# yutiansut/marl-optimal-execution

Measured on AMD Instinct MI355X. Metric: env-steps/sec (whole node), rmsc03 100-agent market ×4096 envs, 1/2/4/8 GPUs, higher is better.
Workload: dtype int64; 1 GPU; rmsc03 x4096 envs per GPU, full episode per step (config build from seeds + the config's session), seeds 123456789+global_env; envs_per_gpu=4096, global_envs=4096, parallelism=envs sharded, dp1, parity_hash=False, env_errors=0, agents_per_env=64, device=AMD Radeon Graphics, cus=256

## Files before the change

### include/mxa.h

```cpp
#ifndef MXA_H
#define MXA_H
#include <stdint.h>
#ifdef __cplusplus
extern "C" {
#endif

typedef struct mxa_handle mxa_handle;

enum { MXA_RMSC03 = 0, MXA_SPARSE_ZI_100 = 1, MXA_SPARSE_ZI_1000 = 2, MXA_MARKETREPLAY = 3, MXA_RMSC03_RL = 4,
       MXA_VALUE_NOISE = 5 ,
       MXA_RMSC01 = 6 ,
       MXA_RMSC02 = 7 ,
       MXA_OBI_RMSC02 = 8 ,
       MXA_RANDOM_FUND_VALUE = 9 ,
       MXA_RANDOM_FUND_DIVERSE = 10 ,
       MXA_HIST_FUND_VALUE = 11 ,
       MXA_HIST_FUND_DIVERSE = 12 ,
       MXA_MARKETREPLAY_RUNNER = 13 ,
       MXA_MARKETREPLAY_TWAP = 14 ,
       MXA_RMSC03_SBMM = 15, MXA_RMSC03_SBMM_POLL = 16,
       MXA_RMSC03_MM = 17 };
enum {
  MXA_OK = 0, MXA_EINVAL = -1, MXA_EHIP = -2, MXA_ENOMEM = -3, MXA_ERANGE = -4
};
// ... 124 lines not shown
  const float* params; int32_t n_layers; int32_t dims[9];
  const double* grid0; int32_t n0; const double* grid1; int32_t n1;
  double nh, q0;
  const double* table;
  int32_t test, enough;
  const double* u; const int64_t* rnd;
  const double* eps;
} mxa_policy;
int mxa_step_policy(mxa_handle* h, int32_t k, int32_t first_zero, const mxa_policy* p, double* d_obs,
                    int32_t* d_flags, int64_t* d_a, double* d_act, double* d_state);
int mxa_set_parity_hash(mxa_handle* h, int32_t enabled);
#define MXA_RL_STATE_WORDS 8
int mxa_write_rl_state(mxa_handle* h, double* device_out);
const char* mxa_build_id(void);

typedef struct {
  int64_t t;
  int32_t price;
  int32_t qty;
} mxa_book_rec;
#define MXA_BL_FUNDAMENTAL (-2147483647 - 1)
int mxa_set_book_log(mxa_handle* h, int32_t cap);
#define MXA_BL_EV_RX (-2147483647 - 1 + 256)
#define MXA_BL_EV_NT (MXA_BL_EV_RX + 256)
#define MXA_BL_EV_PLACE (MXA_BL_EV_RX + 512)
#define MXA_BL_EV_END (MXA_BL_EV_RX + 768)
int mxa_set_exchange_log(mxa_handle* h, int32_t on);
int mxa_read_book_log(mxa_handle* h, int32_t env, mxa_book_rec* out, int64_t cap, int64_t* n);

#include "mxa_snap.h"
#include "mxa_depth.h"
#include "mxa_bars.h"
#include "mxa_variates.h"
#include "mxa_policy_features.h"

int mxa_rng_probe(int32_t device, uint32_t seed, int32_t mode, double a, double b, int32_t n, double* out);
int mxa_math_probe(int32_t device, int32_t mode, const double* x, const double* y, double* out, int64_t n);
int mxa_policy_probe(void* stream, int32_t n, const float* x, const float* params, int32_t n_layers,
                     const int32_t* dims, int32_t test, int32_t enough, const double* u, const int64_t* rnd,
                     const double* eps, float* q, int64_t* a);

#ifdef __cplusplus
}
#endif
#endif
```

### marl-optimal-execution_amd/build_lib.py

```python
import hashlib
import os
import subprocess
import sys
from concurrent.futures import ThreadPoolExecutor

HERE = os.path.dirname(os.path.abspath(__file__))
ROOT = os.path.dirname(HERE)
SRC = os.path.join(HERE, "csrc", "mxa_api.hip")
INST = os.path.join(HERE, "csrc", "mxa_inst.hip")
OUT = os.path.join(HERE, "lib", "libmxa.so")
OBJ = os.path.join(HERE, "build")
N_CONFIGS = 18
DEPS = ["mxa_api.hip", "mxa_inst.hip", "mxa_entry.h", "mxa_kernels.hip", "mxa_layout.h", "mxa_config.h", "glibc_math.h",
        "glibc_math_tables.h", "qnet_wave_device.h", "ddqn_device.h", "mxa_snapshot.h", "mxa_depth_kernels.h",
        "mxa_bars_kernels.h"]
HIPCC = os.environ.get("HIPCC", "/opt/rocm/bin/hipcc")
FLAGS = ["--offload-arch=gfx950", "-O3", "-std=c++20", "-ffp-contract=off", "-fno-fast-math", "-fPIC", "-shared",
         "-Wno-unused-result", "-Wno-unused-value", "-mllvm", "-structurizecfg-skip-uniform-regions"]

CFG_FLAGS = {1: ["-mllvm", "-amdgpu-sched-strategy=max-ilp"], 2: ["-fno-slp-vectorize"],
             3: ["-mllvm", "-amdgpu-sched-strategy=max-ilp"]}


def sources():
    return [os.path.join(HERE, "csrc", d) for d in DEPS] + [os.path.join(ROOT, "include", h) for h in ("mxa.h", "mxa_snap.h", "mxa_depth.h", "mxa_bars.h", "mxa_variates.h", "mxa_policy_features.h", "mxa_state_spec.h")]


def build_id(extra=()):
    h = hashlib.sha256()
    for s in sources():
        with open(s, "rb") as f:
            h.update(f.read())
    h.update(" ".join(FLAGS + list(extra)).encode())
    h.update(repr(sorted(CFG_FLAGS.items())).encode())
    return h.hexdigest()[:16]


def up_to_date():
    if not os.path.exists(OUT):
        return False
    t = os.path.getmtime(OUT)
    return all(os.path.getmtime(s) <= t for s in sources() + [os.path.abspath(__file__)])


def build(force=False, verbose=True, jobs=None):
    if not force and up_to_date():
        return OUT
    os.makedirs(os.path.dirname(OUT), exist_ok=True)
    os.makedirs(OBJ, exist_ok=True)
    inc = ["-I" + os.path.join(HERE, "csrc"), "-I" + os.path.join(ROOT, "include")]
    cflags = [f for f in FLAGS if f != "-shared"] + ["-c"]
    jit = ['-DMXA_JIT_FLAGS="%s"' % " ".join(FLAGS),
           '-DMXA_JIT_CFG_FLAGS="%s"' % ";".join("%d:%s" % (c, " ".join(f)) for c, f in sorted(CFG_FLAGS.items()))]
    units = [([HIPCC] + cflags + ['-DMXA_BUILD_ID="%s"' % build_id()] + jit + inc + [SRC, "-o", os.path.join(OBJ, "mxa_api.o")])]
    for c in range(N_CONFIGS):
        units.append([HIPCC] + cflags + CFG_FLAGS.get(c, []) + ["-DMXA_INST_CFG=%d" % c] + inc +
                     [INST, "-o", os.path.join(OBJ, "mxa_inst_%d.o" % c)])
    if verbose:
# ... 41 lines not shown
```

### marl-optimal-execution_amd/csrc/mxa_api.hip

```cpp
#include <hip/hip_runtime.h>

#include <dlfcn.h>
#include <spawn.h>
#include <sys/stat.h>
#include <sys/wait.h>
#include <unistd.h>

#include <algorithm>
#include <cstddef>
#include <cstdio>
#include <cstdlib>
#include <cstring>
#include <map>
#include <memory>
#include <mutex>
#include <string>
#include <vector>

extern char** environ;

#include "../../include/mxa.h"
#define MXA_API_TU
#include "mxa_kernels.hip"
#include "mxa_entry.h"
// ... 1239 lines not shown
  if (n <= 0 || !out || mode < 0 || mode > 5) return MXA_EINVAL;
  if (hipSetDevice(device) != hipSuccess) return MXA_EHIP;
  DevBuf<double> d_out;
  DevBuf<uint32_t> d_s;
  if (d_out.alloc(n) != hipSuccess || d_s.alloc(MXA_RNG_WORDS) != hipSuccess) return MXA_ENOMEM;
  hipLaunchKernelGGL(mxa_rng_probe_kernel, dim3(1), dim3(64), 0, 0, seed, mode, a, b, n, d_out.p, d_s.p);
  if (hipGetLastError() != hipSuccess) return MXA_EHIP;
  return hipMemcpy(out, d_out, sizeof(double) * n, hipMemcpyDeviceToHost) == hipSuccess ? MXA_OK : MXA_EHIP;
}

int mxa_variate_probe(int32_t device, uint32_t seed, const uint8_t* script, int32_t n, int32_t lookahead, double* out,
                      uint64_t* state) {
  if (n <= 0 || !script || !out || !state || lookahead < 2 || lookahead > 256) return MXA_EINVAL;
  for (int32_t i = 0; i < n; i++)
    if (script[i] > 3) return MXA_EINVAL;
  if (hipSetDevice(device) != hipSuccess) return MXA_EHIP;
  DevBuf<uint8_t> d_script;
  DevBuf<double> d_out;
  DevBuf<uint64_t> d_state, d_tab;
  DevBuf<uint32_t> d_s;
  if (d_script.alloc(n) != hipSuccess || d_out.alloc(2 * (size_t)n) != hipSuccess || d_state.alloc(6 * (size_t)n) != hipSuccess ||
      d_tab.alloc(MXA_VT_BYTES / 8) != hipSuccess || d_s.alloc(2 * MXA_RNG_WORDS) != hipSuccess)
    return MXA_ENOMEM;
  if (hipMemcpy(d_script, script, (size_t)n, hipMemcpyHostToDevice) != hipSuccess ||
      hipMemset(d_tab, 0, MXA_VT_BYTES) != hipSuccess)
    return MXA_EHIP;
  hipLaunchKernelGGL(mxa_variate_probe_kernel, dim3(1), dim3(64), 0, 0, seed, d_script.p, n, lookahead, d_out.p, d_state.p,
                     d_s.p, d_tab.p);
  if (hipGetLastError() != hipSuccess) return MXA_EHIP;
  if (hipMemcpy(out, d_out, sizeof(double) * 2 * (size_t)n, hipMemcpyDeviceToHost) != hipSuccess) return MXA_EHIP;
  return hipMemcpy(state, d_state, sizeof(uint64_t) * 6 * (size_t)n, hipMemcpyDeviceToHost) == hipSuccess ? MXA_OK : MXA_EHIP;
}

int mxa_math_probe(int32_t device, int32_t mode, const double* x, const double* y, double* out, int64_t n) {
  if (n <= 0 || !x || !out) return MXA_EINVAL;
  if (hipSetDevice(device) != hipSuccess) return MXA_EHIP;
  DevBuf<double> dx, dy, dout;
  size_t bytes = sizeof(double) * n;
  if (dx.alloc(n) != hipSuccess || dy.alloc(n) != hipSuccess || dout.alloc(n) != hipSuccess) return MXA_ENOMEM;
  if (hipMemcpy(dx, x, bytes, hipMemcpyHostToDevice) != hipSuccess ||
      hipMemcpy(dy, y ? y : x, bytes, hipMemcpyHostToDevice) != hipSuccess)
    return MXA_EHIP;
  hipLaunchKernelGGL(mxa_math_probe_kernel, dim3((unsigned)((n + 255) / 256)), dim3(256), 0, 0, mode, dx.p, dy.p, dout.p,
                     n);
  if (hipGetLastError() != hipSuccess) return MXA_EHIP;
  return hipMemcpy(out, dout, bytes, hipMemcpyDeviceToHost) == hipSuccess ? MXA_OK : MXA_EHIP;
}

int mxa_policy_probe(void* stream, int32_t n, const float* x, const float* params, int32_t n_layers, const int32_t* dims,
                     int32_t test, int32_t enough, const double* u, const int64_t* rnd, const double* eps, float* q,
                     int64_t* a) {
  if (n <= 0 || !x || !params || !qwave::dims_ok(n_layers, dims) || (!q && !a)) return MXA_EINVAL;
  if (a && !test && (!u || !rnd || !eps)) return MXA_EINVAL;
  MxaPolicyProbe p{};
  p.params = params;
  p.n_layers = n_layers;
  for (int i = 0; i <= n_layers; i++) p.dims[i] = dims[i];
  p.test = test;
  p.enough = enough;
  p.u = u;
  p.rnd = rnd;
  p.eps = eps;
  hipLaunchKernelGGL(mxa_policy_probe_kernel, dim3((unsigned)n), dim3(64), 0, (hipStream_t)stream, p, n, x, q, a);
  return hipGetLastError() == hipSuccess ? MXA_OK : MXA_EHIP;
}

// ... 219 lines not shown
```

### marl-optimal-execution_amd/csrc/mxa_config.h

```cpp
#pragma once
#include <stddef.h>
#include "mxa_layout.h"
#include "../../include/mxa.h"

namespace mxa_cfg {

constexpr int64_t NS = 1000000000LL;
constexpr int64_t MIN = 60 * NS;
constexpr int64_t HOUR = 60 * MIN;

struct Shape {
  int sq, so;
  bool pl;
  int waves;
  int pw;
  int hot;
  int sql = 0;
};
constexpr int sq_lds(int cfg);
constexpr int lat_lds(int cfg);
constexpr Shape shape(int cfg);
constexpr bool is_custom(int cfg);
#ifndef MXA_RMSC03_WAVES
#define MXA_RMSC03_WAVES 4
// ... 79 lines not shown
       : (cfg == MXA_CFG_RANDOM_FUND_VALUE || cfg == MXA_CFG_HIST_FUND_VALUE) ? Shape{96, 5, false, MXA_RFV_WAVES, 6, 0, MXA_RFV_SQL}
       : (cfg == MXA_CFG_RANDOM_FUND_DIVERSE || cfg == MXA_CFG_HIST_FUND_DIVERSE)
           ? Shape{96, MXA_SO_RFD, false, MXA_RFD_WAVES, 8, 0, MXA_RFD_SQL}
                                       : Shape{4, 1, true, 2, 8, MXA_RP_HOT};
}
constexpr int sq_lds(int cfg) { return shape(cfg).sql ? shape(cfg).sql : shape(cfg).sq; }
constexpr bool rp_hdr_lds(int cfg) {
  return cfg == MXA_CFG_MARKETREPLAY || cfg == MXA_CFG_MARKETREPLAY_RUNNER || cfg == MXA_CFG_MARKETREPLAY_TWAP;
}
#ifndef MXA_BOOK_LDS_RFV
#define MXA_BOOK_LDS_RFV 0x34
#endif
constexpr int book_lds(int cfg) {
  return cfg == MXA_CFG_RMSC02 ? MXA_BOOK_LDS_RMSC02
         : (cfg >= MXA_CFG_RANDOM_FUND_VALUE && cfg <= MXA_CFG_HIST_FUND_DIVERSE) ? MXA_BOOK_LDS_RFV
                                                                                 : 0;
}
#ifndef MXA_TEMPER_FILL_MASK
#define MXA_TEMPER_FILL_MASK ((1 << MXA_CFG_RMSC03) | (1 << MXA_CFG_SPARSE_ZI_100) | (1 << MXA_CFG_VALUE_NOISE))
#endif
#ifndef MXA_ONE_ADVANCE_MASK
#define MXA_ONE_ADVANCE_MASK MXA_TEMPER_FILL_MASK
#endif
constexpr bool temper_fill(int cfg) { return (((MXA_TEMPER_FILL_MASK) >> cfg) & 1) != 0; }
constexpr bool one_advance(int cfg) { return (((MXA_ONE_ADVANCE_MASK) >> cfg) & 1) != 0; }
#ifndef MXA_VARIATE_O_MASK
#define MXA_VARIATE_O_MASK (1 << MXA_CFG_RMSC03)
#endif
#ifndef MXA_VARIATE_AGENT_MASK
#define MXA_VARIATE_AGENT_MASK (1 << MXA_CFG_RMSC03)
#endif
constexpr bool variate_o(int cfg) { return (((MXA_VARIATE_O_MASK) >> cfg) & 1) != 0 && !is_custom(cfg); }
constexpr bool variate_agent(int cfg) { return (((MXA_VARIATE_AGENT_MASK) >> cfg) & 1) != 0 && !is_custom(cfg); }
#define MXA_VT_O_BYTES ((2 * 64 + 2) * 8)
#define MXA_VT_BYTES 2048
constexpr size_t lds_bytes(int cfg) {
  return (size_t)sq_lds(cfg) * 64 * (12 + (shape(cfg).pl ? 4 * shape(cfg).pw : 0)) + 512
         + (size_t)shape(cfg).hot * 512
         + 1024
         + (variate_o(cfg) ? MXA_VT_O_BYTES : 0)
         + (size_t)lat_lds(cfg) * 8
         + (rp_hdr_lds(cfg) ? 256 : 0)
         + (size_t)__builtin_popcount(book_lds(cfg)) * shape(cfg).so * 256
         + 256
#ifdef MXA_PROF
         + 1024
#endif
      ;
}

constexpr void base_params(MxaParams& P) {
  P.o_rbar = 1e5;
  P.o_kappa = 1.67e-12;
  P.o_fundvol = 1e-4;
  P.o_lambda = 2.77778e-13;
  P.o_msmean = 1e3;
  P.o_msvar = 5e4;
  P.starting_cash = 10000000;
  P.ex_pipeline = 0;
  P.ex_comp = 0;
  P.stream_history = 10;
  P.mkt_open = 9 * HOUR + 30 * MIN;
}

constexpr void params_rmsc03(MxaParams& P) {
  base_params(P);
// ... 736 lines not shown
```

### marl-optimal-execution_amd/csrc/mxa_kernels.hip

```cpp
#pragma once
#include <hip/hip_runtime.h>
#if defined(MXA_ONLY_RMSC03) && !(defined(MXA_ONLY_CFG) && (MXA_ONLY_CFG == 3 || MXA_ONLY_CFG == 4))
#define MXA_NO_GYM
#endif

#ifndef MXA_HINT_MASK
#define MXA_HINT_MASK ((1 << 0) | (1 << 4))
#endif
#if defined(MXA_INST_CFG)
#define MXA_HINT_ON (((MXA_HINT_MASK) >> (MXA_INST_CFG)) & 1)
#elif defined(MXA_ONLY_RMSC03) && defined(MXA_ONLY_CFG)
#define MXA_HINT_ON (((MXA_HINT_MASK) >> (MXA_ONLY_CFG)) & 1)
#elif defined(MXA_ONLY_RMSC03)
#define MXA_HINT_ON ((MXA_HINT_MASK) & 1)
#else
#define MXA_HINT_ON 0
#endif
#define MXA_EXPECT_(x, v) __builtin_expect(!!(x), v)
#define MXA_PROB_(x, v, p) __builtin_expect_with_probability(!!(x), v, p)
#if MXA_HINT_ON
#define MXA_LIKELY(x) MXA_EXPECT_(x, 1)
#define MXA_UNLIKELY(x) MXA_EXPECT_(x, 0)
#define MXA_RARE(x) MXA_EXPECT_(x, 0)
#define MXA_RARE_P(x, p) MXA_PROB_(x, 1, p)
// ... 188 lines not shown
      a1[q][k] = ok ? A[i + 1] : 0u;
      if (ph == 0) a3[q][k] = ok ? A[i + 397] : 0u;
    }
    a623[q] = on ? A[623] : 0u;
  }
#pragma unroll
  for (int q = 0; q < 2; q++) {
    if (q == 1 && !two) break;
    u32* B = key[q] + (bb[q] & 1) * MXA_MT_N;
    u32 y[11];
#pragma unroll
    for (int k = 0; k < 4; k++) y[k] = a3[q][k] ^ mt_mix(a0[q][k], a1[q][k]);
#pragma unroll
    for (int k = 4; k < 11; k++) y[k] = y[k - 4] ^ mt_mix(a0[q][k], a1[q][k]);
    const u32 b396 = rdl(y[6], 41), b0 = rdl(y[0], 0);
#pragma unroll
    for (int k = 0; k < 11; k++) {
      const int ph = k < 4 ? 0 : k < 8 ? 1 : 2, kk = k - 4 * ph;
      if (kk * 64 + lane < (ph < 2 ? 227 : 169)) B[227 * ph + lane + 64 * kk] = y[k];
    }
    if (lane == 0) B[623] = b396 ^ mt_mix(a623[q], b0);
  }
  wfence();
}
DEV void mt_gen_build(u32* key, int b) { mt_gen_pair(key, b, key, b, false); }

DEV void mt_seed(u32* key, u32 s) {
  const int lane = laneid();
  for (int i = 0; i < MXA_MT_N; i++) {
    if ((i & 63) == lane) key[i] = s;
    s = 1812433253u * (s ^ (s >> 30)) + (u32)i + 1u;
  }
  wfence();
}

DEV u32 mt_temper(u32 y) {
  y ^= (y >> 11);
  y ^= (y << 7) & 0x9d2c5680u;
  y ^= (y << 15) & 0xefc60000u;
  y ^= (y >> 18);
  return y;
}
template <bool B, int W, bool TF>
DEV void rs_fill(RSt<B, W, TF>& r) {
  const int lane = laneid();
  const int q = r.p + lane, b = q / MXA_MT_N;
  const bool ok = b <= r.m && b >= r.m - 1;
  u32 v = 0;
  if (ok) v = r.key[(b & 1) * MXA_MT_N + (q - b * MXA_MT_N)];
  if constexpr (TF) v = mt_temper(v);
  r.lw[lane] = v;
  const u64 okb = __ballot(ok);
  r.lwn = ~okb == 0 ? 64 : __ffsll((unsigned long long)~okb) - 1;
  r.lw0 = r.p;
  if (r.lwn == 0) r.hasg |= 2;
  __threadfence_block();
}
template <bool B, int W, bool TF>
DEV u32 rs_u32(RSt<B, W, TF>& r) {
  if constexpr (W == RS_WIN || W == RS_PTR) {
    if (W == RS_WIN || r.lw) {
      u32 off = (u32)(r.p - r.lw0);
      if (MXA_RARE(off >= (u32)r.lwn)) {
        if constexpr (B) {
          const int blk = r.p / MXA_MT_N;
          while (r.m < blk) {
// ... 2182 lines not shown
    __threadfence_block();
    rs(AF_NUSED, (u32)base);
    return base;
  }

  DEV bool ta_wakeup() {
    PROF_SCOPE(75);
    u32 f = flags();
    if (f & FL_FIRST_WAKE) rs(AF_FLAGS, f & ~FL_FIRST_WAKE);
    if (!(f & FL_HAS_OPEN)) {
      send_ex(msg_make(MK_WHEN_OPEN_REQ, cur_agent));
      send_ex(msg_make(MK_WHEN_CLOSE_REQ, cur_agent));
    }
    f = flags();
    return (f & FL_HAS_OPEN) && (f & FL_HAS_CLOSE) && !(f & FL_MKT_CLOSED);
  }
  DEV i64 wake_frequency(int type) {
    if (type == AG_POVMM) return mm_wake();
    if (type == AG_MOMENTUM) return PC.mom_wake;
    if (type == AG_MKTMAKER) return PC.mk_wake;
    if (type == AG_OBI) return PC.obi_wake;
    if (type == AG_SBMM) return PC.sb_wake;
    if constexpr (RP) {
      if (type == AG_REPLAY) return U(rx->tm[0]) - PC.mkt_open;
      if constexpr (TW) {
        if (type == AG_TWAP) return PC.rl_h0 - PC.mkt_open;
      }
    }
    if constexpr (GYM) {
      if (type == AG_DUMMYRL) return PC.rl_h0 - PC.mkt_open;
    }
    ARS A = agent_rs();
    i64 v = rs_randint(A, 0, 100);
    agent_rs_put(A);
    return v;
  }
  DEV void query_last_trade(const Msg& m) {
    u32 f = flags() | FL_HAS_LAST;
    f = m_dfloat(m) ? (f | FL_LAST_FLOAT) : (f & ~FL_LAST_FLOAT);
    if (f & FL_MKT_CLOSED) f |= FL_DAILY_CLOSE;
    rs(AF_FLAGS, f);
    rs64(AF_LAST_TRADE, (i64)(i32)m.w[5]);
  }
  DEV void ta_receive(const Msg& m, int type) {
    PROF_SCOPE(74);
    u32 f0 = flags();
    bool had = (f0 & FL_HAS_OPEN) && (f0 & FL_HAS_CLOSE);
    switch (m_kind(m)) {
    case MK_WHEN_OPEN:
      rs64(AF_MKT_OPEN, m_i64(m, 1));
      fl_set(FL_HAS_OPEN, true);
      break;
    case MK_WHEN_CLOSE:
      rs64(AF_MKT_CLOSE, m_i64(m, 1));
      fl_set(FL_HAS_CLOSE, true);
      break;
    case MK_EXECUTED: {
      i64 q = m_buy(m) ? (i64)(i32)m.w[2] : -(i64)(i32)m.w[2];
      rs64(AF_SHARES, rg64(AF_SHARES) + q);
      rs64(AF_CASH, rg64(AF_CASH) - q * (i64)(i32)m.w[4]);
      if constexpr (RP) {
        if (type == AG_REPLAY) {
          RPCHK((i32)m.w[5] >= 0 && (i32)m.w[5] < U(rx->L.D), "ta_receive EXECUTED dense", (i32)m.w[5]);
          RpOrder* o = mro() + (i32)m.w[5];
          const RpOrder ov = *o;
          if (U(ov.present)) {
// ... 2742 lines not shown
    this->rs(AF_FLAGS, FL_FIRST_WAKE | FL_AW_SPREAD | FL_AW_TV);
    this->rs(AF_RS_POS, MXA_MT_N);
    this->rs(AF_RS_M, 0);
    const i64 cash = type == AG_VALUE ? E::PC.v_starting_cash : E::PC.starting_cash;
    this->rs64(AF_START_CASH, cash);
    this->rs64(AF_CASH, cash);
    this->rs64(AF_ATIME, E::PC.start);
    this->rs64(AF_COMP, E::PC.default_comp_delay);
  }
  DEV i64 get_wake_time(RS& G, i64 open, i64 close) { return wake_time_of(rs_double(G), open, close); }
  DEV void wake_times_lanes() {
    const MxaParams& P = E::PC;
    wfence();
    for (int a0 = P.first_noise; a0 < P.first_noise + P.n_noise; a0 += 64) {
      const int a = a0 + this->lane;
      if (a < P.first_noise + P.n_noise) {
        u32* rw = (u32*)this->agent_ptr(a);
        const double u = as_d(((u64)rw[AF_WAKEUP_TIME + 1] << 32) | rw[AF_WAKEUP_TIME]);
        const u64 wt = (u64)wake_time_of(u, P.noise_open, P.noise_close);
        rw[AF_WAKEUP_TIME] = (u32)wt;
        rw[AF_WAKEUP_TIME + 1] = (u32)(wt >> 32);
      }
    }
    wfence();
  }
  DEV i64 wake_time_of(double u, i64 open, i64 close) {
    double alpha = 12.0, beta = 0.5;
    double n = (3 / alpha) * u - gm_pow(beta - 0, 3.0);
    double c = n < 0 ? -gm_pow(-n, 1.0 / 3.0) : gm_pow(n, 1.0 / 3.0);
    double mult = c + beta;
    return open + (i64)(mult * (double)(close - open));
  }
  static constexpr bool SEED_TILE = E::LDS_Q >= 64 * 17 * 4;
  DEV void seed_streams(int first) {
    const MxaParams& P = E::PC;
    wfence();
    const int lane = this->lane;
    for (int b = first; b < P.n_streams; b += 64) {
      int s = b + lane;
      if constexpr (SEED_TILE) {
        LDSP u32* tile = (LDSP u32*)this->qk;
        u32 x = s < P.n_streams ? this->rng_key(s)[0] : 0u;
        for (int i0 = 1; i0 < MXA_MT_N; i0 += 16) {
#pragma unroll
          for (int j = 0; j < 16; j++) {
            x = 1812433253u * (x ^ (x >> 30)) + (u32)(i0 + j);
            tile[lane * 17 + j] = x;
          }
          __builtin_amdgcn_wave_barrier();
#pragma unroll
          for (int t = 0; t < 16; t++) {
            const int st = 4 * t + (lane >> 4), w = lane & 15;
            if (b + st < P.n_streams && i0 + w < MXA_MT_N) this->rng_key(b + st)[i0 + w] = tile[st * 17 + w];
          }
          __builtin_amdgcn_wave_barrier();
        }
      } else if (s < P.n_streams) {
        u32* key = this->rng_key(s);
        u32 x = key[0];
        for (int i = 1; i < MXA_MT_N; i++) {
          x = 1812433253u * (x ^ (x >> 30)) + (u32)i;
          key[i] = x;
        }
      }
    }
    wfence();
    if constexpr (SEED_TILE) {
      for (int j = 0; j < E::SQ; j++) this->qset(j, KEY_EMPTY, 0xFFFFFFFFu, true);
      if constexpr (E::QHIER) this->q_rescan();
    }
  }

  DEV void maint_agents() {
    const int n = E::PC.n_agents, lane = this->lane;
    wfence();
    for (int a0 = 0; a0 < n; a0 += 64) {
      const int a = a0 + lane;
      const bool act = a < n;
      u32* rw = (u32*)this->agent_ptr(act ? a : a0);
      const i32 p = act ? (i32)rw[AF_RS_POS] : 0;
      i32 m = act ? (i32)rw[AF_RS_M] : 0;
      const i32 need = (p + MXA_AGENT_LA) / MXA_MT_N;
      for (;;) {
        u64 t = bal(act && m < need);
        if (!t) break;
        const int l1 = ctz64(t);
        t &= t - 1;
        const int l2 = t ? ctz64(t) : l1;
        const int m1 = rdl((u32)m, l1), m2 = rdl((u32)m, l2);
        mt_gen_pair(this->rng_key(4 + a0 + l1), m1 + 1, this->rng_key(4 + a0 + l2), m2 + 1, l2 != l1);
        m += (lane == l1 || lane == l2) ? 1 : 0;
      }
      if (act) rw[AF_RS_M] = (u32)m;
    }
    wfence();
  }

  u64 zi_fb[(E::PC.n_zi + E::PC.n_hbl + 63) / 64 + 1];
  DEV bool zi_fallback(int a) {
    const int i = a - E::PC.first_zi;
    return (zi_fb[i >> 6] >> (i & 63)) & 1;
  }
  DEV void zi_theta_lanes() {
    const MxaParams& P = E::PC;
    constexpr int NQ = 2 * E::PC.zi_qmax;
    static_assert(NQ <= 20, "theta fits the agent record");
    const int lo = P.first_zi, hi = P.first_zi + P.n_zi + P.n_hbl;
    const double sd = __builtin_sqrt(P.zi_sigma_pv);
    const int lane = this->lane;
    for (int a0 = lo; a0 < hi; a0 += 64) {
      for (int j = 0; j < 64 && a0 + j < hi; j += 2)
        mt_gen_pair(this->rng_key(4 + a0 + j), 1, this->rng_key(4 + a0 + j + 1), 1, a0 + j + 1 < hi);
      const int a = a0 + lane;
      const bool act = a < hi;
      const u32* key = this->rng_key(4 + (act ? a : a0));
      i32 p = MXA_MT_N;
      bool cached = false, fb = false;
// ... 389 lines not shown
      double* lat = this->lat();
      i64 total = (i64)n * n, prev = -1;
      bool col = P.config == MXA_CFG_SPARSE_ZI_100;
      i64 nneed = col ? 2 * (i64)n - 1 : (i64)n;
      for (i64 k = 0; k < nneed; k++) {
        i64 d = k < n ? k : (k - n + 1) * (i64)n;
        rs_skip_words(G, 2 * (d - prev - 1));
        double v = rs_uniform(G, P.lat_lo, P.lat_hi);
        if (this->lane == 0) {
          if (d < n) lat[d] = v;
          if (col && d % n == 0) lat[n + d / n] = v;
        }
        prev = d;
      }
      rs_skip_words(G, 2 * (total - prev - 1));
      if (P.config == MXA_CFG_SPARSE_ZI_1000) {
        if (this->lane == 0) lat[0] = 20000.0;
      }
      wfence();
    }
    this->grs_put(0, G);
    seed_streams(1);
    h.rs_pos[1] = h.rs_pos[2] = h.rs_pos[3] = MXA_MT_N;
    h.rs_m[1] = h.rs_m[2] = h.rs_m[3] = 0;
    if constexpr (!E::EXT) {
      RS O = this->grs(1);
      double msv = rs_normal(O, P.o_msmean, __builtin_sqrt(P.o_msvar));
      h.o_msv = rs_randint(O, 0, 2) == 0 ? msv : -msv;
      this->grs_put(1, O);
    }
    rec_init(0, AG_EXCHANGE);
    this->rs64(AF_COMP, P.default_comp_delay);
    this->rec_store();
    for (int a = P.first_mom; a < P.first_mom + P.n_mom; a++) {
      this->rec_load(a);
      ARS A = this->agent_rs();
      this->rs(AF_SIZE, (u32)rs_randint(A, P.mom_min, P.mom_max));
      this->agent_rs_put(A);
      this->rec_store();
    }
    for (int a = P.first_mk; a < P.first_mk + P.n_mk; a++) {
      this->rec_load(a);
      ARS A = this->agent_rs();
      this->rs(AF_SIZE, (u32)(i64)__builtin_rint((double)rs_randint(A, P.mk_min, P.mk_max) / 2));
      this->agent_rs_put(A);
      this->rec_store();
    }
    constexpr bool ZI_LANES = E::PC.n_zi + E::PC.n_hbl > 0;
    if constexpr (ZI_LANES) zi_theta_lanes();
    for (int a = P.first_zi; a < P.first_zi + P.n_zi + P.n_hbl; a++) {
      if (ZI_LANES && !zi_fallback(a)) continue;
      this->rec_load(a);
      ARS A = this->agent_rs();
      double th[20];
      int nq = 2 * P.zi_qmax;
      for (int i = 0; i < 20; i++) th[i] = 0;
      for (int i = 0; i < nq; i++) th[i] = __builtin_rint(rs_normal(A, 0, __builtin_sqrt(P.zi_sigma_pv)));
      for (int i = 1; i < nq; i++) {
        double x = th[i];
        int j = i - 1;
        while (j >= 0 && th[j] < x) {
          th[j + 1] = th[j];
          j--;
        }
        th[j + 1] = x;
      }
      for (int i = 0; i < nq; i++) this->rs(AF_THETA + i, (u32)(i32)th[i]);
      this->agent_rs_put(A);
      this->rec_store();
    }
    for (int k = 0; k < 4; k++) {
      RS r = this->grs(k);
      rs_maint(r);
      this->grs_put(k, r);
    }
    maint_agents();
    if constexpr (E::EXT) {
      const double op = this->efo_price(P.mkt_open);
      h.last_trade = py_round(op);
      h.last_trade_float = 0;
      const i64 t0 = U(this->rx->fs_t[0]), t1 = U(this->rx->fs_t[U(this->rx->fs_n) - 1]);
      h.o_pt = (P.mkt_open >= t0 && P.mkt_open <= t1) ? P.mkt_open : -1;
      h.o_pv = op;
    } else {
      h.last_trade = (i64)P.o_rbar;
      h.last_trade_float = 1;
    }
    this->cur = P.start;
    for (int a = 0; a < n; a++) this->wakeup_at(a, P.start);
    count_base();
    this->save();
    TxRec* R = this->txr();
    for (int i = this->lane; i < P.L.tx_cap; i += 64) {
      TxRec z;
      z.t = 0;
      z.q = 0;
      z.epoch = -1000000;
      R[i] = z;
    }
  }
};

}

// ... 232 lines not shown
__global__ __launch_bounds__(64) void mxa_variate_probe_kernel(uint32_t seed, const uint8_t* script, int n, int cap, double* out,
                                                               uint64_t* state, uint32_t* scratch, uint64_t* tab) {
  for (int pass = 0; pass < 2; pass++) {
    mxa::RSt<true> r;
    r.lw = nullptr;
    r.lw0 = r.lwn = 0;
    r.key = scratch + pass * MXA_RNG_WORDS;
    mxa::mt_seed(r.key, seed);
    r.p = MXA_MT_N;
    r.m = 0;
    r.hasg = 0;
    r.gauss = 0;
    auto none = [](int) {};
    mxa::VtDesc d{0, 0, 0};
    auto put = [&](const mxa::VtDesc& x) { d = x; };
    for (int i = 0; i < n; i++) {
      const int kind = script[i];
      double v;
      if (pass == 0) mxa::rs_maint(r, MXA_AGENT_LA);
      if (kind == 0) v = pass == 0 ? mxa::vt_draw_exponential(r, tab, d, 1.0, put, none, cap) : mxa::rs_exponential(r, 1.0);
      else if (kind == 1) v = pass == 0 ? mxa::vt_draw_gauss<true>(r, tab, d, put, none, cap) : mxa::rs_gauss(r);
      else if (kind == 2) v = (double)mxa::rs_u32(r);
      else v = (double)mxa::rs_randint(r, 0, 100);
      if (__lane_id() == 0) {
        const size_t k = (size_t)pass * n + i;
        out[k] = v;
        state[3 * k] = (uint64_t)(uint32_t)r.p;
        state[3 * k + 1] = (uint64_t)(uint32_t)r.hasg;
        state[3 * k + 2] = mxa::as_u(r.gauss);
      }
    }
  }
}
__global__ void mxa_math_probe_kernel(int mode, const double* x, const double* y, double* out, int64_t n) {
  int64_t i = (int64_t)blockIdx.x * blockDim.x + threadIdx.x;
  if (i >= n) return;
  out[i] = mode == 0 ? gm_log(x[i]) : mode == 1 ? gm_exp(x[i]) : gm_pow(x[i], y[i]);
}
struct MxaPolicyProbe {
  const float* params;
  int32_t n_layers, dims[qwave::kMaxLayers + 1];
  int32_t test, enough;
  const double* u;
  const int64_t* rnd;
  const double* eps;
};
__global__ __launch_bounds__(64) void mxa_policy_probe_kernel(MxaPolicyProbe p, int n, const float* x, float* q, int64_t* a) {
  const int row = blockIdx.x, lane = threadIdx.x;
  if (row >= n) return;
  const int n_in = p.dims[0], n_out = p.dims[p.n_layers];
  float act[qwave::kRegs];
#pragma unroll
  for (int r = 0; r < qwave::kRegs; r++) act[r] = 64 * r + lane < n_in ? x[(size_t)row * n_in + 64 * r + lane] : 0.f;
  qwave::forward(p.params, p.n_layers, p.dims, lane, act);
  if (q != nullptr) {
#pragma unroll
    for (int r = 0; r < qwave::kRegs; r++)
      if (64 * r + lane < n_out) q[(size_t)row * n_out + 64 * r + lane] = act[r];
  }
  if (a == nullptr) return;
  const int greedy = qwave::argmax(act, n_out);
  const int64_t ai = qwave::select(greedy, p.test, p.enough, p.u, p.rnd, p.eps, (size_t)row);
  if (lane == 0) a[row] = ai;
}
#endif
```

### marl-optimal-execution_amd/csrc/mxa_layout.h

```cpp
#pragma once
#include <stdint.h>

#define MXA_MAX_AGENTS 8191
#define MXA_KEY_SHIFT 15
#define MXA_KEY_RCP 0x1FFF
#define MXA_MT_N 624
#define MXA_MT_M 397
#define MXA_RNG_WORDS 1280

enum mxa_config_id { MXA_CFG_RMSC03 = 0, MXA_CFG_SPARSE_ZI_100 = 1, MXA_CFG_SPARSE_ZI_1000 = 2, MXA_CFG_MARKETREPLAY = 3,
                     MXA_CFG_RMSC03_RL = 4, MXA_CFG_VALUE_NOISE = 5, MXA_CFG_RMSC01 = 6,
                     MXA_CFG_RMSC02 = 7, MXA_CFG_OBI_RMSC02 = 8, MXA_CFG_RANDOM_FUND_VALUE = 9,
                     MXA_CFG_RANDOM_FUND_DIVERSE = 10, MXA_CFG_HIST_FUND_VALUE = 11,
                     MXA_CFG_HIST_FUND_DIVERSE = 12, MXA_CFG_MARKETREPLAY_RUNNER = 13,
                     MXA_CFG_MARKETREPLAY_TWAP = 14,
                     MXA_CFG_RMSC03_SBMM = 15, MXA_CFG_RMSC03_SBMM_POLL = 16,
                     MXA_CFG_RMSC03_MM = 17 };

typedef struct {
  double pov;
  int32_t min_order_size;
  int32_t window_size;
  int32_t num_ticks;
  int32_t pad;
  int64_t wake_up_freq;
} MmParams;

enum {
  MK_WAKEUP = 0, MK_WHEN_OPEN_REQ = 1, MK_WHEN_CLOSE_REQ = 2, MK_WHEN_OPEN = 3, MK_WHEN_CLOSE = 4,
  MK_SPREAD_REQ = 5, MK_SPREAD = 6, MK_LAST_REQ = 7, MK_LAST = 8, MK_TV_REQ = 9, MK_TV = 10,
  MK_LIMIT = 11, MK_CANCEL = 12, MK_MODIFY = 13, MK_ACCEPTED = 14, MK_EXECUTED = 15, MK_CANCELLED = 16,
  MK_MKT_CLOSED = 17, MK_MODIFIED = 18, MK_KCANCEL = 19, MK_MARKET_DATA = 20,
  MK_STREAM_REQ = 21, MK_STREAM = 22,
  MK_MD_SUB_REQ = 23, MK_MD_SUB_CANCEL = 24
};
enum { MT_MESSAGE = 1, MT_WAKEUP = 2, MT_CANCEL_ORDER = 3 };

enum { AG_EXCHANGE = 0, AG_ZI = 1, AG_NOISE = 2, AG_VALUE = 3, AG_POVMM = 4, AG_MOMENTUM = 5, AG_REPLAY = 6, AG_DUMMYRL = 7,
       AG_MKTMAKER = 8, AG_HBL = 9, AG_OBI = 10, AG_TWAP = 11, AG_SBMM = 12 };
#define MXA_SB_ID_BASE 0x40000000

enum { ST_RUNNING = 0, ST_DONE = 1, ST_ERROR = 2 };
enum {
  ERR_NONE = 0, ERR_QUEUE_FULL = 1, ERR_BOOK_FULL = 2, ERR_OPEN_FULL = 3, ERR_TX_FULL = 4,
  ERR_PANDAS_NO_TX = 5, ERR_WAKEUP_PAST = 6, ERR_THETA_INDEX = 7, ERR_BAD_CONFIG = 8,
  ERR_RNG_OVERRUN = 9,
  ERR_RP_PRICE = 10,
  ERR_RP_POOL = 11,
  ERR_RP_IDS = 12,
  ERR_RP_KEYERROR = 13,
  ERR_RP_OBS = 14,
  ERR_RP_STOPPING = 15,
  ERR_RP_MODIFY = 16,
  ERR_HBL_WINDOW = 17,
  ERR_HBL_RANGE = 18,
  ERR_FLOAT_PRICE = 19,
  ERR_BOOK_LOG_FULL = 20,
  ERR_MD_NO_UPDATE = 21,
  ERR_MD_SUBS = 22,
  ERR_MD_KEYERROR = 23,
  ERR_MD_SLOT = 24,
  ERR_TWAP_SCHEDULE = 25,
  ERR_TWAP_QUOTE = 26,
  ERR_TWAP_MARKET = 27,
  ERR_SB_MID = 28,
  ERR_ORDER_SIZE = 29,
  ERR_RP_QUOTE_SIZE = 30,
  ERR_ORDER_PRICE = 31
};

typedef struct {
  int64_t cur;
// ... 243 lines not shown
```

### marl-optimal-execution_amd/mxabides/_lib.py

```python
import ctypes
import os

PKG_ROOT = os.path.dirname(os.path.dirname(os.path.abspath(__file__)))
LIB_PATH = os.environ.get("MXA_LIB") or os.path.join(PKG_ROOT, "lib", "libmxa.so")

MXA_RMSC03, MXA_SPARSE_ZI_100, MXA_SPARSE_ZI_1000, MXA_MARKETREPLAY, MXA_RMSC03_RL, MXA_VALUE_NOISE = 0, 1, 2, 3, 4, 5
MXA_RMSC01 = 6
MXA_RMSC02 = 7
MXA_OBI_RMSC02 = 8
MXA_RANDOM_FUND_VALUE = 9
MXA_RANDOM_FUND_DIVERSE = 10
MXA_HIST_FUND_VALUE = 11
MXA_HIST_FUND_DIVERSE = 12
MXA_MARKETREPLAY_RUNNER = 13
MXA_MARKETREPLAY_TWAP = 14
MXA_RMSC03_SBMM = 15
MXA_RMSC03_SBMM_POLL = 16
MXA_RMSC03_MM = 17
CONFIG_IDS = {"rmsc03": MXA_RMSC03, "sparse_zi_100": MXA_SPARSE_ZI_100, "sparse_zi_1000": MXA_SPARSE_ZI_1000,
              "value_noise": MXA_VALUE_NOISE, "rmsc01": MXA_RMSC01, "rmsc02": MXA_RMSC02,
              "obi_rmsc02": MXA_OBI_RMSC02, "random_fund_value": MXA_RANDOM_FUND_VALUE,
              "random_fund_diverse": MXA_RANDOM_FUND_DIVERSE, "hist_fund_value": MXA_HIST_FUND_VALUE,
              "hist_fund_diverse": MXA_HIST_FUND_DIVERSE,
              "marketreplay_runner": MXA_MARKETREPLAY_RUNNER,
# ... 112 lines not shown
    "mxa_step_device": ([_P, _P, _P, _P], _I32),
    "mxa_step_many": ([_P, _I32, _P, _P, _P], _I32),
    "mxa_step_policy": ([_P, _I32, _I32, ctypes.POINTER(Policy), _P, _P, _P, _P, _P], _I32),
    "mxa_set_parity_hash": ([_P, _I32], _I32),
    "mxa_write_rl_state": ([_P, _P], _I32),
    "mxa_build_id": ([], _S),
    "mxa_set_book_log": ([_P, _I32], _I32),
    "mxa_set_exchange_log": ([_P, _I32], _I32),
    "mxa_read_book_log": ([_P, _I32, _P, _I64, _N64], _I32),
    "mxa_rng_probe": ([_I32, _U32, _I32, _D, _D, _I32, _P], _I32),
    "mxa_math_probe": ([_I32, _I32, _P, _P, _P, _I64], _I32),
    "mxa_policy_probe": ([_P, _I32, _P, _P, _I32, _N32, _I32, _I32, _P, _P, _P, _P, _P], _I32),
}
EXPORTS = list(BINDINGS)
SNAPSHOT_BINDINGS = {
    "mxa_snapshot_create": ([_P, _I32, _OUT], _I32),
    "mxa_snapshot_save": ([_P, _P, _P], _I32),
    "mxa_snapshot_restore": ([_P, _P, _P], _I32),
    "mxa_snapshot_info": ([_P, _P], _I32),
    "mxa_snapshot_destroy": ([_P], None),
}
DEPTH_BINDINGS = {
    "mxa_write_depth": ([_P, _I32, _P, _P], _I32),
    "mxa_read_depth": ([_P, _I32, _P, _P], _I32),
}
BARS_BINDINGS = {
    "mxa_write_bars": ([_P, _I64, _I64, _I32, _P, _P], _I32),
    "mxa_read_bars": ([_P, _I64, _I64, _I32, _P, _P], _I32),
    "mxa_bars_from_records": ([_P, _I32, _P, _I64, _P, _I32, _I64, _I64, _I32, _P, _P], _I32),
}
VARIATE_BINDINGS = {
    "mxa_variate_probe": ([_I32, _U32, _P, _I32, _I32, _P, _P], _I32),
}
POLICY_FEATURES_BINDINGS = {
    "mxa_step_policy_spec": ([_P, _I32, _I32, ctypes.POINTER(Policy), ctypes.POINTER(StateSpec), _P, _P, _P, _P, _P],
                             _I32),
}
COUNTER_WORDS = 34
INPLACE_WORDS = 12
RECORD_WORDS = 12

_lib = None


class MxaError(RuntimeError):
    pass


def load():
    global _lib
    if _lib is not None:
        return _lib
    if not os.path.exists(LIB_PATH):
        raise MxaError("libmxa.so not built (%s); run __graft_entry__.build()" % LIB_PATH)
    L = ctypes.CDLL(LIB_PATH)
    for name, (argtypes, restype) in list(BINDINGS.items()) + list(SNAPSHOT_BINDINGS.items()) + list(DEPTH_BINDINGS.items()) \
            + list(BARS_BINDINGS.items()) + list(VARIATE_BINDINGS.items()) + list(POLICY_FEATURES_BINDINGS.items()):
        if hasattr(L, name):
            f = getattr(L, name)
            f.argtypes, f.restype = argtypes, restype
    _lib = L
    return L


def build_id():
    L = load()
    return L.mxa_build_id().decode() if hasattr(L, "mxa_build_id") else "unknown"
```

Measured before the change: 26.94 billion env-steps/s.

## Classify RNG streams and seed/generate only needed Mersenne Twister words

```diff
diff --git a/include/mxa.h b/include/mxa.h
--- a/include/mxa.h
+++ b/include/mxa.h
@@ -180,6 +180,7 @@
 #include "mxa_depth.h"
 #include "mxa_bars.h"
 #include "mxa_variates.h"
+#include "mxa_streams.h"
 #include "mxa_policy_features.h"
 
 int mxa_rng_probe(int32_t device, uint32_t seed, int32_t mode, double a, double b, int32_t n, double* out);
diff --git a/include/mxa_streams.h b/include/mxa_streams.h
--- /dev/null
+++ b/include/mxa_streams.h
@@ -0,0 +1,14 @@
+#ifndef MXA_STREAMS_H
+#define MXA_STREAMS_H
+#include <stdint.h>
+#ifdef __cplusplus
+extern "C" {
+#endif
+
+int mxa_stream_head_probe(int32_t device, uint32_t seed, int32_t head_words, int32_t n, double* out_values,
+                          uint64_t* out_state);
+
+#ifdef __cplusplus
+}
+#endif
+#endif
diff --git a/marl-optimal-execution_amd/build_lib.py b/marl-optimal-execution_amd/build_lib.py
--- a/marl-optimal-execution_amd/build_lib.py
+++ b/marl-optimal-execution_amd/build_lib.py
@@ -23,7 +23,7 @@
 
 
 def sources():
-    return [os.path.join(HERE, "csrc", d) for d in DEPS] + [os.path.join(ROOT, "include", h) for h in ("mxa.h", "mxa_snap.h", "mxa_depth.h", "mxa_bars.h", "mxa_variates.h", "mxa_policy_features.h", "mxa_state_spec.h")]
+    return [os.path.join(HERE, "csrc", d) for d in DEPS] + [os.path.join(ROOT, "include", h) for h in ("mxa.h", "mxa_snap.h", "mxa_depth.h", "mxa_bars.h", "mxa_variates.h", "mxa_streams.h", "mxa_policy_features.h", "mxa_state_spec.h")]
 
 
 def build_id(extra=()):
diff --git a/marl-optimal-execution_amd/csrc/mxa_api.hip b/marl-optimal-execution_amd/csrc/mxa_api.hip
--- a/marl-optimal-execution_amd/csrc/mxa_api.hip
+++ b/marl-optimal-execution_amd/csrc/mxa_api.hip
@@ -1295,6 +1295,22 @@
   return hipMemcpy(state, d_state, sizeof(uint64_t) * 6 * (size_t)n, hipMemcpyDeviceToHost) == hipSuccess ? MXA_OK : MXA_EHIP;
 }
 
+int mxa_stream_head_probe(int32_t device, uint32_t seed, int32_t head_words, int32_t n, double* out_values,
+                          uint64_t* out_state) {
+  if (n <= 0 || !out_values || !out_state || head_words < 2 || head_words > MXA_STREAM_HEAD_WORDS) return MXA_EINVAL;
+  if (hipSetDevice(device) != hipSuccess) return MXA_EHIP;
+  DevBuf<double> d_out;
+  DevBuf<uint64_t> d_state;
+  DevBuf<uint32_t> d_s;
+  if (d_out.alloc((size_t)n) != hipSuccess || d_state.alloc(2 * (size_t)n) != hipSuccess || d_s.alloc(MXA_RNG_WORDS) != hipSuccess)
+    return MXA_ENOMEM;
+  if (hipMemset(d_s, 0, sizeof(uint32_t) * MXA_RNG_WORDS) != hipSuccess) return MXA_EHIP;
+  hipLaunchKernelGGL(mxa_stream_head_probe_kernel, dim3(1), dim3(64), 0, 0, seed, head_words, n, d_out.p, d_state.p, d_s.p);
+  if (hipGetLastError() != hipSuccess) return MXA_EHIP;
+  if (hipMemcpy(out_values, d_out, sizeof(double) * (size_t)n, hipMemcpyDeviceToHost) != hipSuccess) return MXA_EHIP;
+  return hipMemcpy(out_state, d_state, sizeof(uint64_t) * 2 * (size_t)n, hipMemcpyDeviceToHost) == hipSuccess ? MXA_OK : MXA_EHIP;
+}
+
 int mxa_math_probe(int32_t device, int32_t mode, const double* x, const double* y, double* out, int64_t n) {
   if (n <= 0 || !x || !out) return MXA_EINVAL;
   if (hipSetDevice(device) != hipSuccess) return MXA_EHIP;
diff --git a/marl-optimal-execution_amd/csrc/mxa_config.h b/marl-optimal-execution_amd/csrc/mxa_config.h
--- a/marl-optimal-execution_amd/csrc/mxa_config.h
+++ b/marl-optimal-execution_amd/csrc/mxa_config.h
@@ -135,6 +135,32 @@
 #endif
 constexpr bool variate_o(int cfg) { return (((MXA_VARIATE_O_MASK) >> cfg) & 1) != 0 && !is_custom(cfg); }
 constexpr bool variate_agent(int cfg) { return (((MXA_VARIATE_AGENT_MASK) >> cfg) & 1) != 0 && !is_custom(cfg); }
+#ifndef MXA_STREAM_CLASS_MASK
+#define MXA_STREAM_CLASS_MASK (~0)
+#endif
+constexpr int stream_class_of(int type) {
+  switch (type) {
+  case AG_NOISE:
+  case AG_MOMENTUM:
+    return MXA_STREAM_HEAD;
+  case AG_EXCHANGE:
+  case AG_POVMM:
+  case AG_SBMM:
+  case AG_OBI:
+  case AG_DUMMYRL:
+  case AG_REPLAY:
+  case AG_TWAP:
+    return MXA_STREAM_NONE;
+  default:
+    return MXA_STREAM_FULL;
+  }
+}
+constexpr int stream_class(int cfg, int type) {
+  return (((MXA_STREAM_CLASS_MASK) >> cfg) & 1) != 0 ? stream_class_of(type) : MXA_STREAM_FULL;
+}
+#ifndef MXA_STREAM_L_NONE
+#define MXA_STREAM_L_NONE 1
+#endif
 #define MXA_VT_O_BYTES ((2 * 64 + 2) * 8)
 #define MXA_VT_BYTES 2048
 constexpr size_t lds_bytes(int cfg) {
diff --git a/marl-optimal-execution_amd/csrc/mxa_kernels.hip b/marl-optimal-execution_amd/csrc/mxa_kernels.hip
--- a/marl-optimal-execution_amd/csrc/mxa_kernels.hip
+++ b/marl-optimal-execution_amd/csrc/mxa_kernels.hip
@@ -244,6 +244,37 @@
     s = 1812433253u * (s ^ (s >> 30)) + (u32)i + 1u;
   }
   wfence();
+}
+
+DEV bool mt_head_word(int i, int hw) { return i <= hw || (i >= MXA_MT_M && i < MXA_MT_M + hw); }
+DEV void mt_seed_head(u32* key, u32 s, int hw) {
+  const int lane = laneid();
+  for (int i = 0; i < MXA_MT_M + hw; i++) {
+    if ((i & 63) == lane && mt_head_word(i, hw)) key[i] = s;
+    s = 1812433253u * (s ^ (s >> 30)) + (u32)i + 1u;
+  }
+  wfence();
+}
+#define MT_HEAD_BATCH 8
+DEV void mt_gen_heads(u32* const* key, int n, int hw = MXA_STREAM_HEAD_WORDS) {
+  const int lane = laneid();
+  u32 a0[MT_HEAD_BATCH], a1[MT_HEAD_BATCH], a3[MT_HEAD_BATCH];
+#pragma unroll
+  for (int q = 0; q < MT_HEAD_BATCH; q++) {
+    const bool on = q < n && lane < hw;
+    const u32* A = key[q];
+    a0[q] = on ? A[lane] : 0u;
+    a1[q] = on ? A[lane + 1] : 0u;
+    a3[q] = on ? A[lane + MXA_MT_M] : 0u;
+  }
+#pragma unroll
+  for (int q = 0; q < MT_HEAD_BATCH; q++)
+    if (q < n && lane < hw) key[q][MXA_MT_N + lane] = a3[q] ^ mt_mix(a0[q], a1[q]);
+  wfence();
+}
+template <class R>
+DEV void rs_head_guard(R& r, int hw = MXA_STREAM_HEAD_WORDS) {
+  if (MXA_UNLIKELY(r.p > MXA_MT_N + hw)) r.hasg |= 2;
 }
 
 DEV u32 mt_temper(u32 y) {
@@ -2492,6 +2523,7 @@
     }
     ARS A = agent_rs();
     i64 v = rs_randint(A, 0, 100);
+    if (mxa_cfg::stream_class(CFG, type) == MXA_STREAM_HEAD) rs_head_guard(A);
     agent_rs_put(A);
     return v;
   }
@@ -5300,42 +5332,91 @@
     return open + (i64)(mult * (double)(close - open));
   }
   static constexpr bool SEED_TILE = E::LDS_Q >= 64 * 17 * 4;
+  static constexpr int HW = MXA_STREAM_HEAD_WORDS;
+  static_assert(HW <= 64 && HW + MXA_AGENT_LA < MXA_MT_N, "a head is one wave wide and inside block 1's look-ahead");
+  static constexpr bool L_NONE = (MXA_STREAM_L_NONE) && E::PC.lat_mode != 2 &&
+                                 mxa_cfg::stream_class(CFG, AG_EXCHANGE) == MXA_STREAM_NONE;
+  DEV int stream_cls(int s) {
+    if (s < 4) return s == 3 && L_NONE ? MXA_STREAM_NONE : MXA_STREAM_FULL;
+    if (s == 4) return mxa_cfg::stream_class(CFG, AG_EXCHANGE);
+    return mxa_cfg::stream_class(CFG, (int)((const u32*)this->agent_ptr(s - 4))[AF_TYPE]);
+  }
+  DEV void seed_pass(LDSP const u32* pend, int cnt) {
+    const int lane = this->lane;
+    const u32 ent = lane < cnt ? pend[lane] : 1u;
+    const bool anyfull = bal(lane < cnt && !(ent & 1u)) != 0;
+    const int last = anyfull ? MXA_MT_N : MXA_MT_M + HW;
+    if constexpr (SEED_TILE) {
+      LDSP u32* tile = (LDSP u32*)this->qk;
+      u32 x = lane < cnt ? this->rng_key((int)(ent >> 1))[0] : 0u;
+      u32 se[16];
+#pragma unroll
+      for (int t = 0; t < 16; t++) {
+        const int st = 4 * t + (lane >> 4);
+        se[t] = st < cnt ? pend[st] : ~0u;
+      }
+      for (int i0 = 1; i0 < last; i0 += 16) {
+        const bool rnd = anyfull || i0 <= HW || (i0 + 15 >= MXA_MT_M && i0 < MXA_MT_M + HW);
+#pragma unroll
+        for (int j = 0; j < 16; j++) {
+          x = 1812433253u * (x ^ (x >> 30)) + (u32)(i0 + j);
+          if (rnd) tile[lane * 17 + j] = x;
+        }
+        if (!rnd) continue;
+        __builtin_amdgcn_wave_barrier();
+#pragma unroll
+        for (int t = 0; t < 16; t++) {
+          const int st = 4 * t + (lane >> 4), i = i0 + (lane & 15);
+          if (se[t] != ~0u && i < MXA_MT_N && (!(se[t] & 1u) || mt_head_word(i, HW)))
+            this->rng_key((int)(se[t] >> 1))[i] = tile[st * 17 + (lane & 15)];
+        }
+        __builtin_amdgcn_wave_barrier();
+      }
+    } else if (lane < cnt) {
+      u32* key = this->rng_key((int)(ent >> 1));
+      u32 x = key[0];
+      for (int i = 1; i < last; i++) {
+        x = 1812433253u * (x ^ (x >> 30)) + (u32)i;
+        if (!(ent & 1u) || mt_head_word(i, HW)) key[i] = x;
+      }
+    }
+  }
   DEV void seed_streams(int first) {
     const MxaParams& P = E::PC;
     wfence();
     const int lane = this->lane;
+    LDSP u32* pend = this->rwin;
+    int np = 0;
     for (int b = first; b < P.n_streams; b += 64) {
-      int s = b + lane;
-      if constexpr (SEED_TILE) {
-        LDSP u32* tile = (LDSP u32*)this->qk;
-        u32 x = s < P.n_streams ? this->rng_key(s)[0] : 0u;
-        for (int i0 = 1; i0 < MXA_MT_N; i0 += 16) {
-#pragma unroll
-          for (int j = 0; j < 16; j++) {
-            x = 1812433253u * (x ^ (x >> 30)) + (u32)(i0 + j);
-            tile[lane * 17 + j] = x;
-          }
-          __builtin_amdgcn_wave_barrier();
-#pragma unroll
-          for (int t = 0; t < 16; t++) {
-            const int st = 4 * t + (lane >> 4), w = lane & 15;
-            if (b + st < P.n_streams && i0 + w < MXA_MT_N) this->rng_key(b + st)[i0 + w] = tile[st * 17 + w];
-          }
-          __builtin_amdgcn_wave_barrier();
-        }
-      } else if (s < P.n_streams) {
-        u32* key = this->rng_key(s);
-        u32 x = key[0];
-        for (int i = 1; i < MXA_MT_N; i++) {
-          x = 1812433253u * (x ^ (x >> 30)) + (u32)i;
-          key[i] = x;
-        }
-      }
-    }
+      const int s = b + lane;
+      const int cls = s < P.n_streams ? stream_cls(s) : MXA_STREAM_NONE;
+      const u64 mk = bal(cls != MXA_STREAM_NONE);
+      if (cls != MXA_STREAM_NONE)
+        pend[np + __builtin_popcountll(mk & ((1ull << lane) - 1))] = ((u32)s << 1) | (cls == MXA_STREAM_HEAD ? 1u : 0u);
+      np += __builtin_popcountll(mk);
+      __threadfence_block();
+      if (np >= 64) {
+        seed_pass(pend, 64);
+        const u32 e = pend[64 + lane];
+        __threadfence_block();
+        pend[lane] = e;
+        np -= 64;
+        __threadfence_block();
+      }
+    }
+    if (np > 0) seed_pass(pend, np);
     wfence();
     if constexpr (SEED_TILE) {
       for (int j = 0; j < E::SQ; j++) this->qset(j, KEY_EMPTY, 0xFFFFFFFFu, true);
       if constexpr (E::QHIER) this->q_rescan();
+    }
+  }
+  DEV void heads_range(int lo, int n) {
+    for (int a0 = lo; a0 < lo + n; a0 += MT_HEAD_BATCH) {
+      u32* key[MT_HEAD_BATCH];
+#pragma unroll
+      for (int q = 0; q < MT_HEAD_BATCH; q++) key[q] = this->rng_key(4 + min(a0 + q, lo + n - 1));
+      mt_gen_heads(key, min(MT_HEAD_BATCH, lo + n - a0));
     }
   }
 
@@ -5348,9 +5429,22 @@
       u32* rw = (u32*)this->agent_ptr(act ? a : a0);
       const i32 p = act ? (i32)rw[AF_RS_POS] : 0;
       i32 m = act ? (i32)rw[AF_RS_M] : 0;
+      const int cls = act ? mxa_cfg::stream_class(CFG, (int)rw[AF_TYPE]) : MXA_STREAM_FULL;
       const i32 need = (p + MXA_AGENT_LA) / MXA_MT_N;
+      for (u64 t = bal(act && cls == MXA_STREAM_HEAD && m < need); t;) {
+        u32* key[MT_HEAD_BATCH];
+        int k = 0;
+#pragma unroll
+        for (int q = 0; q < MT_HEAD_BATCH; q++) {
+          key[q] = this->rng_key(4 + a0 + (t ? ctz64(t) : 0));
+          k += t ? 1 : 0;
+          t &= t - 1;
+        }
+        mt_gen_heads(key, k);
+      }
+      if (cls != MXA_STREAM_FULL && m < need) m = need;
       for (;;) {
-        u64 t = bal(act && m < need);
+        u64 t = bal(act && cls == MXA_STREAM_FULL && m < need);
         if (!t) break;
         const int l1 = ctz64(t);
         t &= t - 1;
@@ -5806,10 +5900,21 @@
     rec_init(0, AG_EXCHANGE);
     this->rs64(AF_COMP, P.default_comp_delay);
     this->rec_store();
+    constexpr bool MOM_HEAD = mxa_cfg::stream_class(CFG, AG_MOMENTUM) == MXA_STREAM_HEAD;
+    if constexpr (MOM_HEAD) heads_range(P.first_mom, P.n_mom);
     for (int a = P.first_mom; a < P.first_mom + P.n_mom; a++) {
       this->rec_load(a);
       ARS A = this->agent_rs();
-      this->rs(AF_SIZE, (u32)rs_randint(A, P.mom_min, P.mom_max));
+      if constexpr (MOM_HEAD) A.m = 1;
+      i64 size = rs_randint(A, P.mom_min, P.mom_max);
+      if (MOM_HEAD && MXA_UNLIKELY(A.p > MXA_MT_N + HW)) {
+        mt_seed(A.key, A.key[0]);
+        A.p = MXA_MT_N;
+        A.m = 0;
+        A.lw0 = A.lwn = 0;
+        size = rs_randint(A, P.mom_min, P.mom_max);
+      }
+      this->rs(AF_SIZE, (u32)size);
       this->agent_rs_put(A);
       this->rec_store();
     }
@@ -5844,6 +5949,10 @@
       this->rec_store();
     }
     for (int k = 0; k < 4; k++) {
+      if (k == 3 && L_NONE) {
+        h.rs_m[3] = (h.rs_pos[3] + MXA_MT_N) / MXA_MT_N;
+        continue;
+      }
       RS r = this->grs(k);
       rs_maint(r);
       this->grs_put(k, r);
@@ -6142,6 +6251,31 @@
     }
   }
 }
+__global__ __launch_bounds__(64) void mxa_stream_head_probe_kernel(uint32_t seed, int hw, int n, double* out, uint64_t* state,
+                                                                   uint32_t* scratch) {
+  mxa::mt_seed_head(scratch, seed, hw);
+  uint32_t* key[MT_HEAD_BATCH];
+#pragma unroll
+  for (int q = 0; q < MT_HEAD_BATCH; q++) key[q] = scratch;
+  mxa::mt_gen_heads(key, 1, hw);
+  mxa::RSt<false> r;
+  r.lw = nullptr;
+  r.lw0 = r.lwn = 0;
+  r.key = scratch;
+  r.p = MXA_MT_N;
+  r.m = 1;
+  r.hasg = 0;
+  r.gauss = 0;
+  for (int i = 0; i < n; i++) {
+    const double v = (double)mxa::rs_randint(r, 0, 100);
+    mxa::rs_head_guard(r, hw);
+    if (__lane_id() == 0) {
+      out[i] = v;
+      state[2 * i] = (uint64_t)(uint32_t)r.p;
+      state[2 * i + 1] = (uint64_t)(uint32_t)r.hasg;
+    }
+  }
+}
 __global__ void mxa_math_probe_kernel(int mode, const double* x, const double* y, double* out, int64_t n) {
   int64_t i = (int64_t)blockIdx.x * blockDim.x + threadIdx.x;
   if (i >= n) return;
diff --git a/marl-optimal-execution_amd/csrc/mxa_layout.h b/marl-optimal-execution_amd/csrc/mxa_layout.h
--- a/marl-optimal-execution_amd/csrc/mxa_layout.h
+++ b/marl-optimal-execution_amd/csrc/mxa_layout.h
@@ -38,6 +38,8 @@
 
 enum { AG_EXCHANGE = 0, AG_ZI = 1, AG_NOISE = 2, AG_VALUE = 3, AG_POVMM = 4, AG_MOMENTUM = 5, AG_REPLAY = 6, AG_DUMMYRL = 7,
        AG_MKTMAKER = 8, AG_HBL = 9, AG_OBI = 10, AG_TWAP = 11, AG_SBMM = 12 };
+enum { MXA_STREAM_FULL = 0, MXA_STREAM_HEAD = 1, MXA_STREAM_NONE = 2 };
+#define MXA_STREAM_HEAD_WORDS 64
 #define MXA_SB_ID_BASE 0x40000000
 
 enum { ST_RUNNING = 0, ST_DONE = 1, ST_ERROR = 2 };
diff --git a/marl-optimal-execution_amd/mxabides/_lib.py b/marl-optimal-execution_amd/mxabides/_lib.py
--- a/marl-optimal-execution_amd/mxabides/_lib.py
+++ b/marl-optimal-execution_amd/mxabides/_lib.py
@@ -168,6 +168,9 @@
 VARIATE_BINDINGS = {
     "mxa_variate_probe": ([_I32, _U32, _P, _I32, _I32, _P, _P], _I32),
 }
+STREAM_BINDINGS = {
+    "mxa_stream_head_probe": ([_I32, _U32, _I32, _I32, _P, _P], _I32),
+}
 POLICY_FEATURES_BINDINGS = {
     "mxa_step_policy_spec": ([_P, _I32, _I32, ctypes.POINTER(Policy), ctypes.POINTER(StateSpec), _P, _P, _P, _P, _P],
                              _I32),
@@ -191,7 +194,7 @@
         raise MxaError("libmxa.so not built (%s); run __graft_entry__.build()" % LIB_PATH)
     L = ctypes.CDLL(LIB_PATH)
     for name, (argtypes, restype) in list(BINDINGS.items()) + list(SNAPSHOT_BINDINGS.items()) + list(DEPTH_BINDINGS.items()) \
-            + list(BARS_BINDINGS.items()) + list(VARIATE_BINDINGS.items()) + list(POLICY_FEATURES_BINDINGS.items()):
+            + list(BARS_BINDINGS.items()) + list(VARIATE_BINDINGS.items()) + list(STREAM_BINDINGS.items()) + list(POLICY_FEATURES_BINDINGS.items()):
         if hasattr(L, name):
             f = getattr(L, name)
             f.argtypes, f.restype = argtypes, restype
```

Measured after the change: 28.00 billion env-steps/s (median of 6 runs). 1.04x the previous value.
